# Distributed-Deep-Learning/MiniPs

Hardware: AMD Instinct MI355X
Metric: samples/sec (whole node) Criteo-shaped Wide&Deep BSP at 1/2/4/8 MI355X (higher is better)
Workload: dtype bf16; 1 GPU; global_batch=16384, parallelism=ps-dp1 (bsp; single rank: local shards, no collectives), per_gpu_batch=16384, consistency=bsp, world_size=1, backend=none, lookahead=2

## Files before the change

csrc/kernels/gemm_kernels.h:

```cpp
#pragma once
#include <cstdlib>
#include <stdexcept>
#include <string>

#include "common.h"
#include "kernels.h"

namespace minips_k {

typedef __bf16 v8bf __attribute__((ext_vector_type(8)));
typedef unsigned int v4u __attribute__((ext_vector_type(4)));

constexpr int BM = 128, BN = 128;

template <int BK>
struct Lds {
  static constexpr int ROW = BK + 8;
  static constexpr int TR = BM + 16;
  static constexpr int TILE = (BM * ROW > BK * TR) ? BM * ROW : BK * TR;
  static constexpr int CHUNKS = BM * BK / 8 / 256;
};

__device__ __forceinline__ v4s ds_read_tr16(const bf16_t* p) {
  return __builtin_amdgcn_ds_read_tr16_b64_v4i16((__attribute__((address_space(3))) v4s*)(p));
// ... 443 lines not shown
      const int gr = row0 + R, gk = k0 + 8 * c;
      voff = (gr < rows && gk < kend) ? (uint32_t)(((int64_t)gr * ld + gk) * 2) : kOobOffset;
    } else {
      constexpr int CH = ROWS / 8;
      constexpr int RPI = 64 / CH;
      const int kr = RPI * gi + lane / CH;
      const int c = (lane % CH) ^ swz_k(kr);
      const int gk = k0 + kr, gm = row0 + 8 * c;
      voff = (gk < kend && gm < rows) ? (uint32_t)(((int64_t)gk * ld + gm) * 2) : kOobOffset;
    }
    __builtin_amdgcn_raw_ptr_buffer_load_lds(rsrc, (__attribute__((address_space(3))) void*)(S + gi * 512), 16, voff,
                                             0, 0, 0);
  }
}

template <bool KMAJOR, bool PERM, int ROWS>
__device__ __forceinline__ v8s frag2(const bf16_t* S, int row_base, int ks, int lane) {
  const int g = lane >> 4;
  if (!KMAJOR) {
    const int R = row_base + (lane & 15);
    const int c = (4 * ks + g) ^ ((R >> 1) & 7);
    return *reinterpret_cast<const v8s*>(S + R * BK2 + 8 * c);
  } else {
    const int i = lane & 15, q = i >> 2, p = i & 3;
    const int r0 = 32 * ks + (PERM ? 4 * g : 8 * g) + q;
    const int r1 = 32 * ks + (PERM ? 16 + 4 * g : 8 * g + 4) + q;
    const int ch = (row_base >> 3) + (p >> 1), sub = 4 * (p & 1);
    const v4s lo = ds_read_tr16(S + r0 * ROWS + 8 * (ch ^ swz_k(r0)) + sub);
    const v4s hi = ds_read_tr16(S + r1 * ROWS + 8 * (ch ^ swz_k(r1)) + sub);
    return __builtin_shufflevector(lo, hi, 0, 1, 2, 3, 4, 5, 6, 7);
  }
}

template <int TM, int TN, bool A_KM, bool B_KN, int EPI>
__global__ __launch_bounds__(TM * TN / 64) void gemm_v2_kernel(const bf16_t* __restrict__ A,
                                                               const bf16_t* __restrict__ B, int M, int N, int K,
                                                               int lda, int ldb, int k_chunk, EpiArgs ep) {
  constexpr bool PERM = A_KM && B_KN;
  constexpr int WN = TN / 64, NWAVES = (TM / 64) * (TN / 64);
  constexpr int VM_STAGE = (TM / 8 + TN / 8) / NWAVES;
  __shared__ __attribute__((aligned(1024))) bf16_t smem[2][(TM + TN) * BK2];
  static_assert(sizeof(smem) >= sizeof(float) * NWAVES * kScrFloats, "epilogue scratch must fit the staging LDS");
  const int tid = threadIdx.x, lane = tid & 63, wave = tid >> 6;
  const int wm = wave / WN, wn = wave % WN;
  const int tiles_n = (N + TN - 1) / TN, tiles_m = (M + TM - 1) / TM;
  const int nwg = tiles_m * tiles_n;
  int bid = blockIdx.x, ks = blockIdx.z;
  if (ep.zmap && gridDim.z > 1 && gridDim.y == 1) {
    const int W = nwg * (int)gridDim.z, L = bid + nwg * ks;
    const int xcd = L & 7, q = W >> 3, r = W & 7;
    const int w = (xcd < r ? xcd * (q + 1) : r * (q + 1) + (xcd - r) * q) + (L >> 3);
    ks = w / nwg;
    bid = w - ks * nwg;
  } else if (nwg >= 16) {
    int xcd = bid & 7, q = nwg >> 3, r = nwg & 7;
    int base = xcd < r ? xcd * (q + 1) : r * (q + 1) + (xcd - r) * q;
    bid = base + (bid >> 3);
  }
  const int tm = bid / tiles_n, tn = bid % tiles_n;
  const int m0 = tm * TM, n0 = tn * TN;
  {
    const int z = blockIdx.y, zo = z / ep.inner, zi = z - zo * ep.inner;
    A += zo * ep.sa_o + zi * ep.sa_i;
    B += zo * ep.sb_o + zi * ep.sb_i;
    const int64_t co = zo * ep.sc_o + zi * ep.sc_i + (int64_t)ks * ep.sc_split;
    const bool f32 = EPI == kEpiStoreF32 || EPI == kEpiAtomicF32 || EPI == kEpiAccumF32;
    ep.C = f32 ? (void*)((float*)ep.C + co) : (void*)((bf16_t*)ep.C + co);
  }
  const __amdgpu_buffer_rsrc_t ra = __builtin_amdgcn_make_buffer_rsrc((void*)A, (short)0, 0x7ffffff0, 0x00020000);
  const __amdgpu_buffer_rsrc_t rb = __builtin_amdgcn_make_buffer_rsrc((void*)B, (short)0, 0x7ffffff0, 0x00020000);
  const int kb = ks * k_chunk;
  const int ke = min(K, kb + k_chunk);
  const int nt = ke > kb ? (ke - kb + BK2 - 1) / BK2 : 0;

  v4f acc[4][4];
#pragma unroll
  for (int i = 0; i < 4; ++i)
#pragma unroll
    for (int j = 0; j < 4; ++j) acc[i][j] = v4f{0.f, 0.f, 0.f, 0.f};

  if (nt > 0) {
    dma_tile<A_KM, TM, NWAVES>(ra, lda, m0, kb, M, ke, smem[0], wave, lane);
    dma_tile<B_KN, TN, NWAVES>(rb, ldb, n0, kb, N, ke, smem[0] + TM * BK2, wave, lane);
  }
  for (int t = 0; t < nt; ++t) {
    const int cur = t & 1;
    if (t + 1 < nt) {
      const int k1 = kb + (t + 1) * BK2;
      dma_tile<A_KM, TM, NWAVES>(ra, lda, m0, k1, M, ke, smem[cur ^ 1], wave, lane);
      dma_tile<B_KN, TN, NWAVES>(rb, ldb, n0, k1, N, ke, smem[cur ^ 1] + TM * BK2, wave, lane);
      asm volatile("s_waitcnt vmcnt(%0)" ::"n"(VM_STAGE) : "memory");
    } else {
      asm volatile("s_waitcnt vmcnt(0)" ::: "memory");
    }
    __builtin_amdgcn_s_barrier();
    asm volatile("" ::: "memory");
    const bf16_t* SA = smem[cur];
    const bf16_t* SB = smem[cur] + TM * BK2;
#pragma unroll
    for (int ks = 0; ks < BK2 / 32; ++ks) {
      v8s af[4], bfr[4];
#pragma unroll
      for (int i = 0; i < 4; ++i) af[i] = frag2<A_KM, PERM, TM>(SA, wm * 64 + i * 16, ks, lane);
#pragma unroll
      for (int j = 0; j < 4; ++j) bfr[j] = frag2<B_KN, PERM, TN>(SB, wn * 64 + j * 16, ks, lane);
      if (kSetPrio) __builtin_amdgcn_s_setprio(1);
#pragma unroll
      for (int i = 0; i < 4; ++i)
#pragma unroll
        for (int j = 0; j < 4; ++j)
          acc[i][j] = __builtin_amdgcn_mfma_f32_16x16x32_bf16(__builtin_bit_cast(v8bf, af[i]),
                                                              __builtin_bit_cast(v8bf, bfr[j]), acc[i][j], 0, 0, 0);
      if (kSetPrio) __builtin_amdgcn_s_setprio(0);
    }
    asm volatile("s_waitcnt lgkmcnt(0)" ::: "memory");
    __builtin_amdgcn_s_barrier();
    asm volatile("" ::: "memory");
  }
  if (kLdsEpilogue)
    epilogue_lds<EPI, 4>(acc, ep, M, N, m0 + wm * 64, n0 + wn * 64, lane,
                         reinterpret_cast<float*>(&smem[0][0]) + wave * kScrFloats);
  else
    epilogue<EPI>(acc, ep, M, N, m0, n0, wm, wn, lane);
}

inline int gemm_force_tile() {
  static const int v = [] {
    const char* e = std::getenv("MINIPS_GEMM_TILE");
    return e ? std::atoi(e) : 0;
  }();
  return v;
}

template <bool A_KM, bool B_KN, int EPI>
int launch(const bf16_t* A, const bf16_t* B, int M, int N, int K, int lda, int ldb, int split_k,
                  const EpiArgs& ep, int batch, hipStream_t s) {
  int tiles = ((M + BM - 1) / BM) * ((N + BN - 1) / BN);
  const int64_t a_ext = (int64_t)((A_KM ? K : M) - 1) * lda + (A_KM ? M : K);
  const int64_t b_ext = (int64_t)((B_KN ? K : N) - 1) * ldb + (B_KN ? N : K);
  const bool wgrad = A_KM && B_KN;
  const bool v2_ok = a_ext * 2 < 0x7ff00000ll && b_ext * 2 < 0x7ff00000ll;
  const int force = gemm_force_tile();
  if (force != 1 && v2_ok) {
    const int kper = (K + split_k - 1) / split_k;
    const int kc = (kper + BK2 - 1) / BK2 * BK2;
    const int nsplit = (K + kc - 1) / kc;
    const int64_t work = (int64_t)batch * nsplit;
    const int64_t t256 = work * ((M + 255) / 256) * ((N + 255) / 256);
    const int64_t t128 = work * (int64_t)tiles;
    const double eff256 = (double)t256 / (double)(((t256 + 255) / 256) * 256);
    const double eff128 = (double)t128 / (double)(((t128 + 511) / 512) * 512);
// ... 73 lines not shown
```

minips_amd/_native.py:

```python
from __future__ import annotations

import importlib
import os

_loaded: dict = {}


def _load(name: str, what: str, torch_ext: bool = True):
    if name not in _loaded:
        try:
            if torch_ext:
                import torch

            _loaded[name] = importlib.import_module("minips_amd." + name)
        except Exception as e:
            _loaded[name] = e
    mod = _loaded[name]
    if isinstance(mod, Exception):
        state, fix = ("is not built or failed to load", " (or __graft_entry__.build()).") if torch_ext else \
            ("is not built", ".")
        raise RuntimeError(f"minips_amd.{name} ({what}) {state}: {mod!r}. Run `python tools/build.py`{fix}")
    return mod


# ... 3 lines not shown
        return True
    except RuntimeError:
        return False


def kernels():
    return _load("_kernels", "gfx950 HIP kernels")


def evalk():
    return _load("_evalk", "gfx950 HIP evaluation kernels")


def optk():
    return _load("_optk", "gfx950 HIP gradient-clipping kernels")


def ftrlk():
    return _load("_ftrlk", "gfx950 HIP FTRL-Proximal kernel")


def wdftrlk():
    return _load("_wdftrlk", "gfx950 HIP Adagrad + FTRL-Proximal split-row kernel")


def fmk():
    return _load("_fmk", "gfx950 HIP factorization-machine kernels")


def dfmk():
    return _load("_dfmk", "gfx950 HIP DeepFM interaction-term kernels")


def runtime():
    return _load("_runtime", "C++ PS runtime", torch_ext=False)


def kernels_available() -> bool:
    return _available(kernels)


def evalk_available() -> bool:
    return _available(evalk)


def optk_available() -> bool:
    return _available(optk)


def ftrlk_available() -> bool:
    return _available(ftrlk)


def wdftrlk_available() -> bool:
    return _available(wdftrlk)


def fmk_available() -> bool:
    return _available(fmk)


def dfmk_available() -> bool:
    return _available(dfmk)


def native_dir() -> str:
    return os.path.dirname(os.path.abspath(__file__))
```

minips_amd/models/widedeep.py:

```python
from __future__ import annotations

from dataclasses import dataclass, field

import torch

from .. import ops
from ..ps.comm import Comm
from ..utils import streams
from ..utils.metrics import phase, traced
from .layers import Replayer, SideStream
from .feeder import LookaheadPlans


@dataclass
class WideDeepConfig:
    cards: list = field(default_factory=lambda: list(__import__(
        "minips_amd.data.synthetic", fromlist=["CRITEO_KAGGLE_CARDS"]).CRITEO_KAGGLE_CARDS))
    n_dense: int = 13
    emb_dim: int = 32
    row_width: int = 36
    hidden: tuple = (1024, 512, 256)
    lr_dense: float = 1e-3
    lr_sparse: float = 0.02
    consistency: str = "bsp"
    staleness: int = 0
    transport: str = "auto"
    dense_transport: str | None = None
    max_batch: int = 16384
    seed: int = 0
    bucket_mb: float = 0.0
    wide_optimizer: str = "adagrad"
    wide_alpha: float = 0.1
    wide_beta: float = 1.0
    wide_l1: float = 0.0
    wide_l2: float = 0.0
    wide_grad_scale: float = 1.0
    fm_term: bool = False

    def __post_init__(self):
# ... 6 lines not shown
        if self.wide_optimizer == "ftrl" and self.transport == "onesided":
            raise ValueError("wide_optimizer 'ftrl' needs transport 'collective' (the one-sided owners apply the "
                             "row-wise Adagrad only)")
        if self.fm_term and "onesided" in (self.transport, self.dense_transport):
            raise ValueError("fm_term needs transport 'collective' (the DeepFM term is not built for the one-sided "
                             "transport)")
        if self.fm_term and not 1 <= self.emb_dim <= 64:
            raise ValueError(f"fm_term: emb_dim is {self.emb_dim}, expected 1 <= emb_dim <= 64")

    @property
    def F(self):
        return len(self.cards)

    @property
    def in_dim(self):
        k = self.F * self.emb_dim + self.n_dense + 1
        return (k + 7) // 8 * 8


_PLAN_AT = {1: "dgrad", 2: "dgrad"}
_DENSE_CLOCK_ON_SIDE = False


_K1_ALIGN = 64
_WGRAD_BLOCKS = 256


_DENSE_ON_SIDE = True
_W1_LATE = False
_ADAM_AFTER_DGRAD = True
_ROWIDX = True
_REPLAY = True
_HEAD_DEFER = True


def _wgrad(dH, H, Gw, sink=None):
    return ops.linear_wgrad(dH, H, Gw, blocks=_WGRAD_BLOCKS, defer=sink)


def _align(n, a=8):
    return (n + a - 1) // a * a


def _table_maker(comm, engine):
    from ..engine import create_table

    if engine is not None:
        return lambda kind, **kw: engine.table(engine.create_table(kind, **kw))
    ids = iter(range(1 << 20))
    return lambda kind, **kw: create_table(comm, kind, table_id=next(ids), **kw)


class WideDeep(LookaheadPlans):
    def __init__(self, cfg: WideDeepConfig, comm: Comm, engine=None):
        self.cfg = cfg
        self.comm = comm
        dev = comm.device
        F, D = cfg.F, cfg.emb_dim
        self.num_rows = int(sum(cfg.cards))
        bases = [sum(cfg.cards[:f]) for f in range(F)]
        make = _table_maker(comm, engine)
        onesided = cfg.transport == "onesided"
        self.emb = make("sparse", num_rows=self.num_rows, width=cfg.row_width, optimizer="rowwise_adagrad",
                        lr=cfg.lr_sparse, model=cfg.consistency, staleness=cfg.staleness, transport=cfg.transport,
                        split=D, init_std=0.01, seed=cfg.seed, columns=(bases, cfg.cards), pull_dtype=torch.bfloat16,
                        **({"max_keys": cfg.max_batch * F} if onesided else {}),
                        **(dict(wide_optimizer="ftrl", wide_lr=cfg.wide_alpha, ftrl_beta=cfg.wide_beta, l1=cfg.wide_l1,
                                l2=cfg.wide_l2, ftrl_grad_scale=cfg.wide_grad_scale)
                           if cfg.wide_optimizer == "ftrl" else {}))
        self.emb.shard[:, D:].zero_()
        self.k_in = [cfg.F * cfg.emb_dim + cfg.n_dense, *cfg.hidden[:-1]]
        self.k_pad = [_align(self.k_in[0] + 1, _K1_ALIGN),
                      *self.k_in[1:]]
        self.layout = {}
        off = 0
        for i, n_out in enumerate(cfg.hidden):
            self.layout[f"W{i + 1}"] = (off, (n_out, self.k_pad[i]))
            off += _align(n_out * self.k_pad[i], 64)
            if i > 0:
                self.layout[f"b{i + 1}"] = (off, (n_out,))
                off += _align(n_out, 64)
        self.layout["w4"] = (off, (cfg.hidden[-1] + 8,))
        off += cfg.hidden[-1] + 8
        self.n_params = off
        starts = [self.layout[f"W{i + 1}"][0] for i in range(len(cfg.hidden))]
        bucketed = cfg.bucket_mb > 0 and cfg.dense_transport == "collective" and comm.world > 1
        self.dense = make("dense", n_params=self.n_params, optimizer="adam", lr=cfg.lr_dense, model=cfg.consistency,
                          staleness=cfg.staleness, transport=cfg.dense_transport,
                          **(dict(buckets=starts, bucket_mb=cfg.bucket_mb) if bucketed else {}))
        self._wbucket = [self.dense.bucket_for_layer(x) for x in starts] if bucketed else None
        self.dense.load_full(self._init_dense(dev))
        self._bufs = {}
        self._side = SideStream(dev)
        self._replay = Replayer(self._side) if self._side.stream is not None else None

    def _init_dense(self, dev):
        g = torch.Generator(device="cpu")
        g.manual_seed(self.cfg.seed + 17)
        full = torch.zeros(self.n_params, dtype=torch.float32)
        for i in range(len(self.cfg.hidden)):
            w = self.view(full, f"W{i + 1}")
            ops.kaiming_uniform_(w[:, : self.k_in[i]], self.k_in[i], g)
            w[:, self.k_in[i]:] = 0
        h = self.cfg.hidden[-1]
        ops.kaiming_uniform_(self.view(full, "w4")[:h], h, g)
        return full.to(dev)

    def view(self, buf: torch.Tensor, name: str) -> torch.Tensor:
        key = (buf.data_ptr(), buf.dtype, name)
        views = self.__dict__.setdefault("_views", {})
        v = views.get(key)
        if v is None:
            off, shape = self.layout[name]
            n = 1
            for s in shape:
                n *= s
            v = buf[off: off + n].view(shape)
            if buf.is_cuda:
                if len(views) > 256:
                    views.clear()
                views[key] = v
        return v

    def _buffers(self, B):
        if B not in self._bufs:
            dev, cfg = self.comm.device, self.cfg
            bf = dict(dtype=torch.bfloat16, device=dev)
            h1, h2, h3 = cfg.hidden

            X = torch.zeros(B, self.k_pad[0], **bf)
            X[:, self.k_in[0]] = 1.0

            self._bufs[B] = dict(
                X=X, H1=torch.empty(B, h1, **bf), H2=torch.empty(B, h2, **bf),
                H3=torch.empty(B, h3, **bf), dH3=torch.empty(B, h3, **bf), dH2=torch.empty(B, h2, **bf),
                dH1=torch.empty(B, h1, **bf),
                dX=torch.empty(B, cfg.F * cfg.emb_dim, **bf),
                wide=torch.empty(B, dtype=torch.float32, device=dev),
                dwide=torch.empty(B, dtype=torch.float32, device=dev),
                loss=torch.zeros(1, dtype=torch.float32, device=dev),
            )
            if cfg.fm_term:
                self._bufs[B]["S"] = torch.empty(B, cfg.emb_dim, dtype=torch.float32, device=dev)
        return self._bufs[B]

    def _forward(self, b, P):
        ops.linear_fwd(b["X"], self.view(P, "W1"), None, "relu", out=b["H1"])
        ops.linear_fwd(b["H1"], self.view(P, "W2"), self.view(P, "b2"), "relu", out=b["H2"])
        ops.linear_fwd(b["H2"], self.view(P, "W3"), self.view(P, "b3"), "relu", out=b["H3"])

    def forward(self, dense, keys, rows, plan):
        B = dense.shape[0]
        b = self._buffers(B)
        pend_side = self.__dict__.pop("_side_pending", None)
        if pend_side is not None:
            streams.current(self.comm.device).wait_event(pend_side[1])
        P = self.dense.get()
        F, D = self.cfg.F, self.cfg.emb_dim
        ops.wd_assemble(dense, rows, plan.inv, F, D, b["X"], b["wide"], ones_col=self.k_in[0])
        if self.cfg.fm_term:
            ops.wd_fm_forward(b["X"], F, D, b["wide"], b["S"])
        self._forward(b, P)
        h = self.cfg.hidden[-1]
        w4 = self.view(P, "w4").float()
        return b["H3"].float() @ w4[:h] + w4[h] + b["wide"]

    def _eval_buffers(self, B):
        bufs = self.__dict__.setdefault("_ebufs", {})
        if B not in bufs:
            dev, cfg = self.comm.device, self.cfg
            bf = dict(dtype=torch.bfloat16, device=dev)
            X = torch.zeros(B, self.k_pad[0], **bf)
            X[:, self.k_in[0]] = 1.0
            bufs[B] = dict(X=X, wide=torch.empty(B, dtype=torch.float32, device=dev),
                           **{f"H{i + 1}": torch.empty(B, n, **bf) for i, n in enumerate(cfg.hidden)})
            if cfg.fm_term:
                bufs[B]["S"] = torch.empty(B, cfg.emb_dim, dtype=torch.float32, device=dev)
        return bufs[B]

    def evaluate(self, batches, evaluator=None) -> dict:
        from ..utils.evalmetrics import BinaryEvaluator

        cfg = self.cfg
        if "onesided" in (cfg.transport, cfg.dense_transport):
            raise NotImplementedError("WideDeep.evaluate: the onesided transport is not supported (its Gets move the "
                                      "SSP gate's staleness statistics and need a clock); evaluate on 'collective'")
        ev = evaluator if evaluator is not None else BinaryEvaluator(self.comm.device)
        F, D, h = cfg.F, cfg.emb_dim, cfg.hidden[-1]
        pend_side = self.__dict__.get("_side_pending")
        if pend_side is not None:
            streams.current(self.comm.device).wait_event(pend_side[1])
        P = self.dense.get()
        w4 = self.view(P, "w4")
        for dense, keys, labels in batches:
            b = self._eval_buffers(dense.shape[0])
            rows, plan = self.emb.get(keys, plan=self.emb.plan(keys))
            ops.wd_assemble(dense, rows, plan.inv, F, D, b["X"], b["wide"], ones_col=self.k_in[0])
            if cfg.fm_term:
                ops.wd_fm_forward(b["X"], F, D, b["wide"], b["S"])
            self._forward(b, P)
            ev.update_head(b["H3"], w4[:h], w4[h:h + 1], b["wide"], labels)
        ev.reduce(self.comm)
        return ev.result()

    @traced("wd.train_step")
    def train_step(self, dense, keys, labels, next_keys=None, next_on_plan_stream: bool = False) -> torch.Tensor:
        cfg = self.cfg
        B = dense.shape[0]
        F, D = cfg.F, cfg.emb_dim
        h = cfg.hidden[-1]
        b = self._buffers(B)
        plan = self._take_plan(keys)

        def issue_next(point):
            if next_keys is not None and point == _PLAN_AT[min(2, self.comm.world)]:
                nk = next_keys() if callable(next_keys) else next_keys
                self.prefetch(nk, keys_on_plan_stream=next_on_plan_stream)

        with phase("wd.plan_next"):
            issue_next("start")
        pend_side = self.__dict__.pop("_side_pending", None)
        if pend_side is not None and pend_side[0] is not None:
            streams.current(self.comm.device).wait_event(pend_side[0])
        ph = phase("wd.get_assemble")
        ph.__enter__()
        src = self.emb.get_source(keys, plan=plan)
        if src is not None:
            plan, table, index, base = src
            rowidx = plan.csr[4] if plan.csr is not None and len(plan.csr) >= 5 and _ROWIDX else None
            ops.wd_assemble_tab(dense, table, index, base, plan.inv, F, D, b["X"], b["wide"], ones_col=self.k_in[0],
                                zero=b["loss"], rowidx=rowidx)
        else:
            rows, plan = self.emb.get(keys, plan=plan)
            ops.wd_assemble(dense, rows, plan.inv, F, D, b["X"], b["wide"], ones_col=self.k_in[0], zero=b["loss"])
        if cfg.fm_term:
            ops.wd_fm_forward(b["X"], F, D, b["wide"], b["S"])
        if pend_side is not None:
            streams.current(self.comm.device).wait_event(pend_side[1])
        ph.__exit__(None, None, None)
        ph = phase("wd.fwd_head")
        ph.__enter__()
        G = self.dense.grad
        P = self.dense.get()
        scale = 1.0 / (B * self.comm.world)
        w4, gw4 = self.view(P, "w4"), self.view(G, "w4")
        sink = self.dense.slab_sink() if hasattr(self.dense, "slab_sink") else None
        side = self._side
        defer = _HEAD_DEFER and side.stream is not None
        rp = self._replay if (self._replay is not None and _REPLAY and self._wbucket is None
                              and streams.DELAY_US <= 0 and not torch.cuda.is_current_stream_capturing()) else None
        key = (B, P.data_ptr(), G.data_ptr(), sink is not None, defer)
        if rp is not None:
            rp(("fwd",) + key, lambda: self._forward(b, P))
        else:
            self._forward(b, P)
        ops.wd_head(b["H3"], w4[:h], w4[h:h + 1], b["wide"], labels, b["dH3"], gw4[:h], gw4[h:h + 1],
                    b["dwide"], b["loss"], self.view(G, "b3"), scale, defer_fold=defer)
        ph.__exit__(None, None, None)
        ph = phase("wd.bwd_dense")
        ph.__enter__()
        issue_next("head")
        fold = (B, h, gw4[:h], gw4[h:h + 1], b["loss"], self.view(G, "b3")) if defer else None
        if rp is not None:
            rp(("bwd",) + key, lambda: self._backward_chain(b, P, G, sink, side, fold))
        else:
            self._backward_chain(b, P, G, sink, side, fold)
        sorted_rows = plan.csr is not None and len(plan.csr) >= 3 and plan.csr[2] is not None
        if sorted_rows:
            ops.linear_dgrad(b["dH1"], self.view(P, "W1"), n_cols=F * D, out=b["dX"].view(B * F, D),
                             perm=plan.csr[2], seg=D)
        else:
            ops.linear_dgrad(b["dH1"], self.view(P, "W1"), n_cols=F * D, out=b["dX"])
        w_read = side.point() if _ADAM_AFTER_DGRAD and self.comm.world == 1 else None
        if cfg.fm_term:
            ops.wd_fm_backward(b["X"], b["S"], b["dwide"], b["dX"], F, D, perm=plan.csr[2] if sorted_rows else None)
        if _W1_LATE:
            with side.fork():
                _wgrad(b["dH1"], b["X"], self.view(G, "W1"), sink)
        pipe = getattr(self.dense, "pipe", None)
        dense_early = _DENSE_CLOCK_ON_SIDE and pipe is not None and pipe.async_ and side.stream is not None
        if dense_early:
            with side.fork():
                self.dense.add()
                self.dense.clock()
        issue_next("dgrad")
        ph.__exit__(None, None, None)
        ph = phase("wd.emb_push")
        ph.__enter__()
        dXe = b["dX"].view(B * F, D) if sorted_rows else b["dX"]
        self.emb.add_lookup_grads(plan, dXe, b["dwide"], F, D, sorted_rows=sorted_rows)
        self.emb.clock()
        issue_next("push")
        ph.__exit__(None, None, None)
        ph = phase("wd.dense_clock")
        ph.__enter__()
# ... 60 lines not shown
```

minips_amd/ops/__init__.py:

```python
from __future__ import annotations

import math

import torch

from .._native import dfmk, evalk, fmk, ftrlk, kernels, optk, wdftrlk

EPI_STORE_F32 = 0
EPI_ATOMIC_F32 = 1
EPI_BIAS_RELU_BF16 = 2
EPI_BIAS_BF16 = 3
EPI_STORE_BF16 = 4
EPI_RELU_MASK_BF16 = 5
EPI_BIAS_GELU_BF16 = 6
EPI_BIAS_GELU_AUX_BF16 = 7
EPI_GELU_GRAD_BF16 = 8
EPI_PERM_ROWS_BF16 = 9
EPI_BIAS_GELU_DAUX_BF16 = 13
EPI_MUL_AUX_BF16 = 14
_L2E = 1.4426950408889634


def _gelu_grad(u):
    k, c = 0.7978845608, 0.044715
    t = torch.tanh(k * (u + c * u ** 3))
    return 0.5 * (1 + t) + 0.5 * u * (1 - t * t) * k * (1 + 3 * c * u * u)


def _gpu(t: torch.Tensor) -> bool:
    return t.is_cuda


_NO_STRIDES: list = []
_REC = None


class recording:

    def __init__(self, lst):
# ... 502 lines not shown
                                  zero, rowidx)
        return X, wide_logit
    U = int(inv.max()) + 1 if inv.numel() else 0
    rows = table[index[:U] - base].to(torch.bfloat16)
    return wd_assemble(dense, rows, inv, F, D, X, wide_logit, ones_col, zero)


def wd_head(H, w, b0, wide_logit, labels, dH, dw, db, dwide, loss_sum, dH_colsum=None, grad_scale=1.0,
            defer_fold=False):
    if _gpu(H):
        kernels().wd_head(H, w, b0, wide_logit, labels, dH, dw, db, dwide, loss_sum, dH_colsum, float(grad_scale),
                          bool(defer_fold))
        return
    h = H.float()
    z = h @ w.float() + b0.float() + wide_logit
    y = (labels > 0.5).float()
    p = torch.sigmoid(z)
    dz = (p - y) * grad_scale
    dwide.copy_(dz)
    db += dz.sum()
    loss_sum += (torch.clamp_min(z, 0) - z * y + torch.log1p(torch.exp(-z.abs()))).sum()
    g = torch.where(h > 0, dz.unsqueeze(1) * w.float().unsqueeze(0), torch.zeros_like(h)).to(torch.bfloat16)
    dH.copy_(g)
    dw += (dz.unsqueeze(1) * h).sum(0)
    if dH_colsum is not None:
        dH_colsum += g.float().sum(0)


def wd_head_fold(B, Hd, dw, db, loss_sum, dH_colsum=None):
    if _gpu(dw):
        (kernels() if _REC is None else _REC.lst).wd_head_fold(int(B), int(Hd), dw, db, loss_sum, dH_colsum)


def _wd_fm_check(X, F, D):
    if not 1 <= D <= 64 or F < 1:
        raise RuntimeError(f"wd_fm: D is {D} and F is {F}, expected 1 <= D <= 64 and F >= 1")
    if X.dim() != 2 or X.shape[1] < F * D:
        raise RuntimeError(f"wd_fm: X has shape {tuple(X.shape)}, expected [B, >= F * D = {F * D}]")


def wd_fm_forward(X, F, D, wide, S=None, blocks=0):
    F, D, B = int(F), int(D), X.shape[0]
    if S is None:
        S = torch.empty(B, D, dtype=torch.float32, device=X.device)
    if _gpu(X):
        dfmk().wd_fm_forward(X, F, D, wide, S, int(blocks))
        return S
    _wd_fm_check(X, F, D)
    v = X[:, : F * D].float().reshape(B, F, D)
    s = v.sum(1)
    S.copy_(s)
    wide += 0.5 * (s * s - (v * v).sum(1)).sum(1)
    return S


def wd_fm_backward(X, S, dwide, dX, F, D, perm=None, blocks=0):
    F, D, B = int(F), int(D), X.shape[0]
    if _gpu(X):
        dfmk().wd_fm_backward(X, S, dwide, perm, dX, F, D, int(blocks))
        return dX
    _wd_fm_check(X, F, D)
    n = B * F
    if dX.numel() != n * D or not dX.is_contiguous():
        raise RuntimeError(f"wd_fm_backward: dX {tuple(dX.shape)}, expected {n * D} contiguous elements")
    v = X[:, : F * D].float().reshape(n, D)
    dx = dX.view(n, D)
# ... 600 lines not shown
```

Before: 48.70 million samples/s.

## Fuse layer-3 GEMM with Wide&Deep head and BCE loss into one tail kernel

Adds a HIP kernel that computes the last hidden layer (H2·W3ᵀ + b3, ReLU), the output head, the BCE loss and its gradient in one pass. H3 is never written to global memory, and per-block partial sums (dw4, db4, loss, b3 column sums) are reduced by a separate fold kernel launched on the side stream. This removes the layer-3 GEMM launch, the H3 round trip and the separate head kernel. In exchange, each block recomputes the full 256-wide N tile, and the design relies on a partials buffer and on restricted shapes (N a multiple of 64, at most 256). The GEMM main loop is factored into a macro so the new kernel can reuse it.

```diff
diff --git a/csrc/bindings/wdtail_py.cpp b/csrc/bindings/wdtail_py.cpp
--- /dev/null
+++ b/csrc/bindings/wdtail_py.cpp
@@ -0,0 +1,108 @@
+#include <ATen/hip/impl/HIPGuardImplMasqueradingAsCUDA.h>
+#include <ATen/hip/impl/HIPStreamMasqueradingAsCUDA.h>
+#include <torch/extension.h>
+
+#include "../kernels/wdtail.h"
+#include "tensor_access.h"
+
+namespace {
+
+using namespace minips_access;
+using OptTensor = c10::optional<at::Tensor>;
+using DeviceGuard = c10::hip::HIPGuardMasqueradingAsCUDA;
+
+void check_n(int64_t N, const char* what) {
+  TORCH_CHECK(N >= 64 && N <= minips_k::kTailMaxN && N % 64 == 0, what, " ", N, ", expected a multiple of 64 up to ",
+              minips_k::kTailMaxN);
+}
+
+int64_t wd_tail(const at::Tensor& H2, const at::Tensor& W3, const at::Tensor& b3, const at::Tensor& w4,
+                const at::Tensor& b4, const at::Tensor& wide, const at::Tensor& labels, at::Tensor& dH3,
+                at::Tensor& dwide, at::Tensor& partials, const OptTensor& H3_out, double grad_scale, int64_t tile) {
+  TORCH_CHECK(H2.dim() == 2 && W3.dim() == 2, "H2 and W3 must be matrices ([B, K] and [N, K])");
+  const int64_t B = H2.size(0), K = H2.size(1), N = W3.size(0);
+  check_n(N, "W3 has N =");
+  TORCH_CHECK(tile == 0 || tile == 64 || tile == 128, "tile is ", tile, ", expected 0, 64 or 128");
+  TORCH_CHECK(B >= 1, "H2 has shape ", H2.sizes(), ", expected at least one row");
+  TORCH_CHECK(W3.size(1) == K, "W3 has shape ", W3.sizes(), ", expected [N, ", K, "] (H2's columns)");
+  const int64_t ldh = B > 1 ? H2.stride(0) : K, ldw = W3.stride(0);
+  DeviceGuard gd(gpu_of(H2, "H2"));
+  const bf16_t* hp = dev_rows<bf16_t>(H2, "H2", B, K);
+  const bf16_t* wp = dev_rows<bf16_t>(W3, "W3", N, K);
+  TORCH_CHECK(minips_k::tail_shape_ok(B, N, K, ldh, ldw), "H2 has shape ", H2.sizes(), " (ld ", ldh, "), W3 ",
+              W3.sizes(), " (ld ", ldw, "): K and both leading dimensions must be multiples of 8, below 2 GiB each");
+  aligned16(H2, "H2");
+  aligned16(W3, "W3");
+  TORCH_CHECK(b3.dim() == 1 && b3.numel() == N, "b3 has shape ", b3.sizes(), ", expected [", N, "]");
+  TORCH_CHECK(w4.dim() == 1 && w4.numel() == N, "w4 has shape ", w4.sizes(), ", expected [", N, "]");
+  TORCH_CHECK(b4.dim() == 1 && b4.numel() == 1, "b4 has shape ", b4.sizes(), ", expected [1]");
+  TORCH_CHECK(wide.dim() == 1 && wide.numel() == B, "wide has shape ", wide.sizes(), ", expected [", B, "]");
+  TORCH_CHECK(labels.dim() == 1 && labels.numel() == B, "labels has shape ", labels.sizes(), ", expected [", B, "]");
+  TORCH_CHECK(dH3.dim() == 2 && dH3.size(0) == B && dH3.size(1) == N, "dH3 has shape ", dH3.sizes(), ", expected [", B,
+              ", ", N, "]");
+  TORCH_CHECK(dwide.dim() == 1 && dwide.numel() == B, "dwide has shape ", dwide.sizes(), ", expected [", B, "]");
+  const int64_t rows = minips_k::tail_blocks(B, tile == 0 ? minips_k::kTailDefaultTM : (int)tile), NP = 2 * N + 2;
+  TORCH_CHECK(partials.dim() == 2 && partials.size(1) == NP && partials.size(0) >= rows, "partials has shape ",
+              partials.sizes(), ", expected [>= ", rows, ", ", NP, "]");
+  if (present(H3_out))
+    TORCH_CHECK(H3_out->dim() == 2 && H3_out->size(0) == B && H3_out->size(1) == N, "H3_out has shape ",
+                H3_out->sizes(), ", expected [", B, ", ", N, "]");
+  const bf16_t* b3p = dev<bf16_t>(b3, "b3", N);
+  const bf16_t* w4p = dev<bf16_t>(w4, "w4", N);
+  const bf16_t* b4p = dev<bf16_t>(b4, "b4", 1);
+  const float* wdp = dev<float>(wide, "wide", B);
+  const float* lbp = dev<float>(labels, "labels", B);
+  bf16_t* dhp = dev<bf16_t>(dH3, "dH3", B * N);
+  float* dwp = dev<float>(dwide, "dwide", B);
+  float* pp = dev<float>(partials, "partials", rows * NP);
+  bf16_t* h3p = dev_opt<bf16_t>(H3_out, "H3_out", B * N);
+  aligned16(dH3, "dH3");
+  if (present(H3_out)) aligned16(*H3_out, "H3_out");
+  const auto d = H2.device();
+  TORCH_CHECK(W3.device() == d && b3.device() == d && w4.device() == d && b4.device() == d && wide.device() == d &&
+                  labels.device() == d && dH3.device() == d && dwide.device() == d && partials.device() == d &&
+                  (!present(H3_out) || H3_out->device() == d),
+              "W3, b3, w4, b4, wide, labels, dH3, dwide, partials and H3_out must be on H2's device");
+  return minips_k::wd_tail(hp, ldh, wp, ldw, b3p, w4p, b4p, wdp, lbp, dhp, dwp, pp, h3p, B, (int)N, (int)K,
+                           (float)grad_scale, (int)tile, stream_of(H2));
+}
+
+void wd_tail_fold(const at::Tensor& partials, int64_t nblocks, int64_t N, at::Tensor& dw4, at::Tensor& db4,
+                  at::Tensor& loss_sum, const OptTensor& colsum_b3) {
+  check_n(N, "N is");
+  TORCH_CHECK(nblocks >= 1 && nblocks <= minips_k::kTailMaxBlocks, "nblocks is ", nblocks,
+              ", expected 1 <= nblocks <= ", minips_k::kTailMaxBlocks);
+  const int64_t NP = 2 * N + 2;
+  TORCH_CHECK(partials.dim() == 2 && partials.size(1) == NP && partials.size(0) >= nblocks, "partials has shape ",
+              partials.sizes(), ", expected [>= nblocks = ", nblocks, ", ", NP, "]");
+  TORCH_CHECK(dw4.dim() == 1 && dw4.numel() == N, "dw4 has shape ", dw4.sizes(), ", expected [", N, "]");
+  TORCH_CHECK(db4.dim() == 1 && db4.numel() == 1, "db4 has shape ", db4.sizes(), ", expected [1]");
+  TORCH_CHECK(loss_sum.dim() == 1 && loss_sum.numel() == 1, "loss_sum has shape ", loss_sum.sizes(), ", expected [1]");
+  if (present(colsum_b3))
+    TORCH_CHECK(colsum_b3->dim() == 1 && colsum_b3->numel() == N, "colsum_b3 has shape ", colsum_b3->sizes(),
+                ", expected [", N, "]");
+  DeviceGuard gd(gpu_of(partials, "partials"));
+  const float* pp = dev<float>(partials, "partials", nblocks * NP);
+  float* dwp = dev<float>(dw4, "dw4", N);
+  float* dbp = dev<float>(db4, "db4", 1);
+  float* lp = dev<float>(loss_sum, "loss_sum", 1);
+  float* cp = dev_opt<float>(colsum_b3, "colsum_b3", N);
+  const auto d = partials.device();
+  TORCH_CHECK(dw4.device() == d && db4.device() == d && loss_sum.device() == d &&
+                  (!present(colsum_b3) || colsum_b3->device() == d),
+              "dw4, db4, loss_sum and colsum_b3 must be on partials' device");
+  minips_k::wd_tail_fold(pp, (int)nblocks, (int)N, dwp, dbp, lp, cp, stream_of(partials));
+}
+
+}
+
+PYBIND11_MODULE(TORCH_EXTENSION_NAME, m) {
+  m.doc() = "minips_amd fused Wide & Deep MLP tail: layer-3 GEMM + head + BCE forward/backward (gfx950)";
+  m.def("wd_tail", &wd_tail, py::arg("H2"), py::arg("W3"), py::arg("b3"), py::arg("w4"), py::arg("b4"),
+        py::arg("wide"), py::arg("labels"), py::arg("dH3"), py::arg("dwide"), py::arg("partials"), py::arg("H3_out"),
+        py::arg("grad_scale"), py::arg("tile"));
+  m.def("wd_tail_fold", &wd_tail_fold, py::arg("partials"), py::arg("nblocks"), py::arg("N"), py::arg("dw4"),
+        py::arg("db4"), py::arg("loss_sum"), py::arg("colsum_b3"));
+  m.attr("MAX_N") = minips_k::kTailMaxN;
+  m.attr("MAX_BLOCKS") = minips_k::kTailMaxBlocks;
+}
diff --git a/csrc/kernels/gemm_kernels.h b/csrc/kernels/gemm_kernels.h
--- a/csrc/kernels/gemm_kernels.h
+++ b/csrc/kernels/gemm_kernels.h
@@ -499,6 +499,41 @@
   }
 }
 
+#define MINIPS_GEMM_V2_MAIN_LOOP(TM, TN, ra, rb, lda, ldb, M, N, m0, n0, kb, ke, nt, smem, wave, lane, wm, wn, acc) \
+  if (nt > 0) {                                                                                                    \
+    dma_tile<A_KM, TM, NWAVES>(ra, lda, m0, kb, M, ke, smem[0], wave, lane);                                       \
+    dma_tile<B_KN, TN, NWAVES>(rb, ldb, n0, kb, N, ke, smem[0] + TM * BK2, wave, lane);                            \
+  }                                                                                                                \
+  for (int t = 0; t < nt; ++t) {                                                                                   \
+    const int cur = t & 1;                                                                                         \
+    if (t + 1 < nt) {                                                                                              \
+      const int k1 = kb + (t + 1) * BK2;                                                                           \
+      dma_tile<A_KM, TM, NWAVES>(ra, lda, m0, k1, M, ke, smem[cur ^ 1], wave, lane);                               \
+      dma_tile<B_KN, TN, NWAVES>(rb, ldb, n0, k1, N, ke, smem[cur ^ 1] + TM * BK2, wave, lane);                    \
+                                                                       \
+      asm volatile("s_waitcnt vmcnt(%0)" ::"n"(VM_STAGE) : "memory");                                              \
+    } else {                                                                                                       \
+      asm volatile("s_waitcnt vmcnt(0)" ::: "memory");                                                             \
+    }                                                                                                              \
+    __builtin_amdgcn_s_barrier();                                                                                  \
+    asm volatile("" ::: "memory");                                                                                 \
+    const bf16_t* SA = smem[cur];                                                                                  \
+    const bf16_t* SB = smem[cur] + TM * BK2;                                                                       \
+    _Pragma("unroll") for (int ks = 0; ks < BK2 / 32; ++ks) {                                                      \
+      v8s af[4], bfr[4];                                                                                           \
+      _Pragma("unroll") for (int i = 0; i < 4; ++i) af[i] = frag2<A_KM, PERM, TM>(SA, wm * 64 + i * 16, ks, lane); \
+      _Pragma("unroll") for (int j = 0; j < 4; ++j) bfr[j] = frag2<B_KN, PERM, TN>(SB, wn * 64 + j * 16, ks, lane); \
+      if (kSetPrio) __builtin_amdgcn_s_setprio(1);                \
+      _Pragma("unroll") for (int i = 0; i < 4; ++i) _Pragma("unroll") for (int j = 0; j < 4; ++j) acc[i][j] =      \
+          __builtin_amdgcn_mfma_f32_16x16x32_bf16(__builtin_bit_cast(v8bf, af[i]), __builtin_bit_cast(v8bf, bfr[j]), \
+                                                  acc[i][j], 0, 0, 0);                                             \
+      if (kSetPrio) __builtin_amdgcn_s_setprio(0);                                                                 \
+    }                                                                                                              \
+    asm volatile("s_waitcnt lgkmcnt(0)" ::: "memory");                                                             \
+    __builtin_amdgcn_s_barrier();                     \
+    asm volatile("" ::: "memory");                                                                                 \
+  }
+
 template <int TM, int TN, bool A_KM, bool B_KN, int EPI>
 __global__ __launch_bounds__(TM * TN / 64) void gemm_v2_kernel(const bf16_t* __restrict__ A,
                                                                const bf16_t* __restrict__ B, int M, int N, int K,
@@ -546,44 +581,7 @@
 #pragma unroll
     for (int j = 0; j < 4; ++j) acc[i][j] = v4f{0.f, 0.f, 0.f, 0.f};
 
-  if (nt > 0) {
-    dma_tile<A_KM, TM, NWAVES>(ra, lda, m0, kb, M, ke, smem[0], wave, lane);
-    dma_tile<B_KN, TN, NWAVES>(rb, ldb, n0, kb, N, ke, smem[0] + TM * BK2, wave, lane);
-  }
-  for (int t = 0; t < nt; ++t) {
-    const int cur = t & 1;
-    if (t + 1 < nt) {
-      const int k1 = kb + (t + 1) * BK2;
-      dma_tile<A_KM, TM, NWAVES>(ra, lda, m0, k1, M, ke, smem[cur ^ 1], wave, lane);
-      dma_tile<B_KN, TN, NWAVES>(rb, ldb, n0, k1, N, ke, smem[cur ^ 1] + TM * BK2, wave, lane);
-      asm volatile("s_waitcnt vmcnt(%0)" ::"n"(VM_STAGE) : "memory");
-    } else {
-      asm volatile("s_waitcnt vmcnt(0)" ::: "memory");
-    }
-    __builtin_amdgcn_s_barrier();
-    asm volatile("" ::: "memory");
-    const bf16_t* SA = smem[cur];
-    const bf16_t* SB = smem[cur] + TM * BK2;
-#pragma unroll
-    for (int ks = 0; ks < BK2 / 32; ++ks) {
-      v8s af[4], bfr[4];
-#pragma unroll
-      for (int i = 0; i < 4; ++i) af[i] = frag2<A_KM, PERM, TM>(SA, wm * 64 + i * 16, ks, lane);
-#pragma unroll
-      for (int j = 0; j < 4; ++j) bfr[j] = frag2<B_KN, PERM, TN>(SB, wn * 64 + j * 16, ks, lane);
-      if (kSetPrio) __builtin_amdgcn_s_setprio(1);
-#pragma unroll
-      for (int i = 0; i < 4; ++i)
-#pragma unroll
-        for (int j = 0; j < 4; ++j)
-          acc[i][j] = __builtin_amdgcn_mfma_f32_16x16x32_bf16(__builtin_bit_cast(v8bf, af[i]),
-                                                              __builtin_bit_cast(v8bf, bfr[j]), acc[i][j], 0, 0, 0);
-      if (kSetPrio) __builtin_amdgcn_s_setprio(0);
-    }
-    asm volatile("s_waitcnt lgkmcnt(0)" ::: "memory");
-    __builtin_amdgcn_s_barrier();
-    asm volatile("" ::: "memory");
-  }
+  MINIPS_GEMM_V2_MAIN_LOOP(TM, TN, ra, rb, lda, ldb, M, N, m0, n0, kb, ke, nt, smem, wave, lane, wm, wn, acc)
   if (kLdsEpilogue)
     epilogue_lds<EPI, 4>(acc, ep, M, N, m0 + wm * 64, n0 + wn * 64, lane,
                          reinterpret_cast<float*>(&smem[0][0]) + wave * kScrFloats);
diff --git a/csrc/kernels/wdtail.h b/csrc/kernels/wdtail.h
--- /dev/null
+++ b/csrc/kernels/wdtail.h
@@ -0,0 +1,30 @@
+#pragma once
+
+#include <hip/hip_runtime.h>
+#include <stdint.h>
+
+namespace minips_k {
+
+constexpr int kTailMaxN = 256;
+constexpr int kTailMaxBlocks = 256;
+constexpr int kTailDefaultTM = 128;
+
+inline bool tail_shape_ok(int64_t B, int64_t N, int64_t K, int64_t ldh, int64_t ldw) {
+  constexpr int64_t kMaxElems = 0x7ff00000ll >> 1;
+  return B >= 1 && N >= 64 && N <= kTailMaxN && N % 64 == 0 && K >= 8 && K % 8 == 0 && ldh >= K && ldw >= K &&
+         ldh % 8 == 0 && ldw % 8 == 0 && (B - 1) * ldh + K < kMaxElems && (N - 1) * ldw + K < kMaxElems;
+}
+
+inline int tail_blocks(int64_t B, int tm) {
+  const int64_t tiles = (B + tm - 1) / tm;
+  return (int)(tiles < kTailMaxBlocks ? tiles : kTailMaxBlocks);
+}
+
+int wd_tail(const uint16_t* H2, int64_t ldh, const uint16_t* W3, int64_t ldw, const uint16_t* b3, const uint16_t* w4,
+            const uint16_t* b4, const float* wide, const float* labels, uint16_t* dH3, float* dwide, float* partials,
+            uint16_t* H3_out, int64_t B, int N, int K, float grad_scale, int tm, hipStream_t stream);
+
+void wd_tail_fold(const float* partials, int nblocks, int N, float* dw4, float* db4, float* loss_sum,
+                  float* colsum_b3, hipStream_t stream);
+
+}
diff --git a/csrc/kernels/wdtail.hip b/csrc/kernels/wdtail.hip
--- /dev/null
+++ b/csrc/kernels/wdtail.hip
@@ -0,0 +1,261 @@
+#include "wdtail.h"
+
+#include <stdexcept>
+#include <string>
+
+#include "gemm_kernels.h"
+
+namespace minips_k {
+namespace {
+
+constexpr int kTailTN = 256;
+
+__device__ __forceinline__ void tail_store_slice(const v4f (&v)[4], float* __restrict__ scr, bf16_t* __restrict__ dst,
+                                                 int B, int N, int row0, int nb, int lane) {
+  const int col_l = lane & 15, row_q = (lane >> 4) * 4;
+#pragma unroll
+  for (int j = 0; j < 4; ++j)
+#pragma unroll
+    for (int r = 0; r < 4; ++r) scr[(row_q + r) * kScrPitch + j * 16 + col_l] = v[j][r];
+  __builtin_amdgcn_wave_barrier();
+#pragma unroll
+  for (int ro = 0; ro < 2; ++ro) {
+    const int rr = ro * 8 + (lane >> 3), c8 = (lane & 7) * 8;
+    const int row = row0 + rr, col = nb + c8;
+    const float4 lo = *reinterpret_cast<const float4*>(scr + rr * kScrPitch + c8);
+    const float4 hi = *reinterpret_cast<const float4*>(scr + rr * kScrPitch + c8 + 4);
+    if (row >= B || col >= N) continue;
+    auto pk = [](float a, float b) { return (__float_as_uint(a) >> 16) | (__float_as_uint(b) & 0xffff0000u); };
+    *reinterpret_cast<uint4*>(dst + (int64_t)row * N + col) =
+        make_uint4(pk(lo.x, lo.y), pk(lo.z, lo.w), pk(hi.x, hi.y), pk(hi.z, hi.w));
+  }
+  __builtin_amdgcn_wave_barrier();
+}
+
+template <int TM>
+__global__ __launch_bounds__(TM * 4, 2) void wd_tail_kernel(const bf16_t* __restrict__ H2,
+                                                         const bf16_t* __restrict__ W3, int B, int N, int K, int ldh,
+                                                         int ldw,
+                                                         const bf16_t* __restrict__ b3, const bf16_t* __restrict__ w4,
+                                                         const bf16_t* __restrict__ b4, const float* __restrict__ wide,
+                                                         const float* __restrict__ labels, bf16_t* __restrict__ dH3,
+                                                         float* __restrict__ dwide, float* __restrict__ partials,
+                                                         bf16_t* __restrict__ H3_out, float scale, int ntiles) {
+  constexpr bool A_KM = false, B_KN = false, PERM = false;
+  constexpr int TN = kTailTN, WMS = TM / 64, NWAVES = WMS * (TN / 64);
+  constexpr int VM_STAGE = (TM / 8 + TN / 8) / NWAVES;
+  __shared__ __attribute__((aligned(1024))) bf16_t smem[2][(TM + TN) * BK2];
+  const int tid = threadIdx.x, lane = tid & 63, wave = tid >> 6;
+  const int wm = wave / (TN / 64), wn = wave % (TN / 64);
+  const int col_l = lane & 15, row_q = (lane >> 4) * 4;
+  float* const lds = reinterpret_cast<float*>(&smem[0][0]);
+  float* const scr = lds + wave * kScrFloats;
+  float* const zpart = lds + NWAVES * kScrFloats;
+  float* const dzs = zpart + 4 * TM;
+  float* const red = dzs + TM;
+  float* const red_s = red + 2 * WMS * TN;
+  static_assert(sizeof(smem) >= sizeof(float) * (NWAVES * kScrFloats + 5 * TM + 2 * WMS * TN + 2 * NWAVES),
+                "the epilogue's scratch must fit the staging LDS");
+
+  const __amdgpu_buffer_rsrc_t ra = __builtin_amdgcn_make_buffer_rsrc((void*)H2, (short)0, 0x7ffffff0, 0x00020000);
+  const __amdgpu_buffer_rsrc_t rb = __builtin_amdgcn_make_buffer_rsrc((void*)W3, (short)0, 0x7ffffff0, 0x00020000);
+  const int nt = (K + BK2 - 1) / BK2;
+
+  float wc[4], bc[4], dwl[4], csl[4];
+#pragma unroll
+  for (int j = 0; j < 4; ++j) {
+    const int col = wn * 64 + j * 16 + col_l;
+    wc[j] = col < N ? bf2f(w4[col]) : 0.f;
+    bc[j] = col < N ? bf2f(b3[col]) : 0.f;
+    dwl[j] = 0.f;
+    csl[j] = 0.f;
+  }
+  const float bias4 = bf2f(b4[0]);
+  float dbl = 0.f, lossl = 0.f;
+
+  for (int tile = blockIdx.x; tile < ntiles; tile += gridDim.x) {
+    const int m0 = tile * TM;
+    v4f acc[4][4];
+#pragma unroll
+    for (int i = 0; i < 4; ++i)
+#pragma unroll
+      for (int j = 0; j < 4; ++j) acc[i][j] = v4f{0.f, 0.f, 0.f, 0.f};
+    MINIPS_GEMM_V2_MAIN_LOOP(TM, TN, ra, rb, ldh, ldw, B, N, m0, 0, 0, K, nt, smem, wave, lane, wm, wn, acc)
+
+#pragma unroll
+    for (int i = 0; i < 4; ++i)
+#pragma unroll
+      for (int j = 0; j < 4; ++j)
+#pragma unroll
+        for (int r = 0; r < 4; r += 2) {
+          const uint32_t p = pack_bf2(fmaxf(acc[i][j][r] + bc[j], 0.f), fmaxf(acc[i][j][r + 1] + bc[j], 0.f));
+          acc[i][j][r] = __uint_as_float(p << 16);
+          acc[i][j][r + 1] = __uint_as_float(p & 0xffff0000u);
+        }
+    if (H3_out) {
+#pragma unroll
+      for (int i = 0; i < 4; ++i)
+        tail_store_slice(acc[i], scr, H3_out, B, N, m0 + wm * 64 + i * 16, wn * 64, lane);
+    }
+#pragma unroll
+    for (int i = 0; i < 4; ++i)
+#pragma unroll
+      for (int r = 0; r < 4; ++r) {
+        float s = 0.f;
+#pragma unroll
+        for (int j = 0; j < 4; ++j) s += acc[i][j][r] * wc[j];
+        s += __shfl_xor(s, 1, 64);
+        s += __shfl_xor(s, 2, 64);
+        s += __shfl_xor(s, 4, 64);
+        s += __shfl_xor(s, 8, 64);
+        if (col_l == 0) zpart[wn * TM + wm * 64 + i * 16 + row_q + r] = s;
+      }
+    __syncthreads();
+    if (tid < TM) {
+      const int row = m0 + tid;
+      float dz = 0.f;
+      if (row < B) {
+        const float z = ((zpart[tid] + zpart[TM + tid]) + zpart[2 * TM + tid]) + zpart[3 * TM + tid];
+        const float zz = z + bias4 + wide[row];
+        const float label = labels[row] > 0.5f ? 1.f : 0.f;
+        const float p = sigmoidf_(zz);
+        dz = (p - label) * scale;
+        dwide[row] = dz;
+        dbl += dz;
+        lossl += fmaxf(zz, 0.f) - zz * label + log1pf(__expf(-fabsf(zz)));
+      }
+      dzs[tid] = dz;
+    }
+    __syncthreads();
+
+#pragma unroll
+    for (int i = 0; i < 4; ++i) {
+      const float4 d4 = *reinterpret_cast<const float4*>(dzs + wm * 64 + i * 16 + row_q);
+      const float dz[4] = {d4.x, d4.y, d4.z, d4.w};
+      v4f g[4];
+#pragma unroll
+      for (int j = 0; j < 4; ++j)
+#pragma unroll
+        for (int r = 0; r < 4; r += 2) {
+          const float h0 = acc[i][j][r], h1 = acc[i][j][r + 1];
+          const uint32_t p = pack_bf2(h0 > 0.f ? dz[r] * wc[j] : 0.f, h1 > 0.f ? dz[r + 1] * wc[j] : 0.f);
+          g[j][r] = __uint_as_float(p << 16);
+          g[j][r + 1] = __uint_as_float(p & 0xffff0000u);
+          dwl[j] += dz[r] * h0;
+          dwl[j] += dz[r + 1] * h1;
+          csl[j] += g[j][r];
+          csl[j] += g[j][r + 1];
+        }
+      tail_store_slice(g, scr, dH3, B, N, m0 + wm * 64 + i * 16, wn * 64, lane);
+    }
+    __syncthreads();
+  }
+
+#pragma unroll
+  for (int j = 0; j < 4; ++j) {
+    dwl[j] += __shfl_xor(dwl[j], 16, 64);
+    dwl[j] += __shfl_xor(dwl[j], 32, 64);
+    csl[j] += __shfl_xor(csl[j], 16, 64);
+    csl[j] += __shfl_xor(csl[j], 32, 64);
+    if (lane < 16) {
+      red[wm * TN + wn * 64 + j * 16 + lane] = dwl[j];
+      red[(WMS + wm) * TN + wn * 64 + j * 16 + lane] = csl[j];
+    }
+  }
+  dbl = warp_sum(dbl);
+  lossl = warp_sum(lossl);
+  if (lane == 0) {
+    red_s[wave] = dbl;
+    red_s[NWAVES + wave] = lossl;
+  }
+  __syncthreads();
+  float* const prow = partials + (int64_t)blockIdx.x * (2 * N + 2);
+  for (int c = tid; c < N; c += TM * 4) {
+    float a = 0.f, b = 0.f;
+#pragma unroll
+    for (int w = 0; w < WMS; ++w) {
+      a += red[w * TN + c];
+      b += red[(WMS + w) * TN + c];
+    }
+    prow[c] = a;
+    prow[N + c] = b;
+  }
+  if (tid == 0) {
+    float a = 0.f, b = 0.f;
+#pragma unroll
+    for (int w = 0; w < NWAVES; ++w) {
+      a += red_s[w];
+      b += red_s[NWAVES + w];
+    }
+    prow[2 * N] = a;
+    prow[2 * N + 1] = b;
+  }
+}
+
+constexpr int kTailFoldCols = 32, kTailFoldChunks = 16;
+__global__ __launch_bounds__(kTailFoldCols* kTailFoldChunks) void wd_tail_fold_kernel(
+    const float* __restrict__ partials, int nb, int N, float* dw, float* colsum, float* db, float* loss_sum) {
+  __shared__ float red[kTailFoldChunks][kTailFoldCols + 1];
+  const int NP = 2 * N + 2;
+  const int cl = threadIdx.x % kTailFoldCols, ch = threadIdx.x / kTailFoldCols;
+  const int c = blockIdx.x * kTailFoldCols + cl;
+  const int per = (nb + kTailFoldChunks - 1) / kTailFoldChunks;
+  const int r0 = ch * per, r1 = min(nb, r0 + per);
+  float acc = 0.f;
+  if (c < NP) {
+    for (int r = r0; r < r1; r += 8) {
+      float v[8];
+#pragma unroll
+      for (int k = 0; k < 8; ++k) v[k] = r + k < r1 ? partials[(int64_t)(r + k) * NP + c] : 0.f;
+#pragma unroll
+      for (int k = 0; k < 8; ++k) acc += v[k];
+    }
+  }
+  red[ch][cl] = acc;
+  __syncthreads();
+  if (ch != 0 || c >= NP) return;
+  float tot = 0.f;
+#pragma unroll
+  for (int k = 0; k < kTailFoldChunks; ++k) tot += red[k][cl];
+  if (c < N) dw[c] += tot;
+  else if (c < 2 * N) {
+    if (colsum) colsum[c - N] += tot;
+  } else if (c == 2 * N) *db += tot;
+  else *loss_sum += tot;
+}
+
+}
+
+int wd_tail(const uint16_t* H2, int64_t ldh, const uint16_t* W3, int64_t ldw, const uint16_t* b3, const uint16_t* w4,
+            const uint16_t* b4, const float* wide, const float* labels, uint16_t* dH3, float* dwide, float* partials,
+            uint16_t* H3_out, int64_t B, int N, int K, float grad_scale, int tm, hipStream_t stream) {
+  if (B <= 0) return 0;
+  if (!tail_shape_ok(B, N, K, ldh, ldw))
+    throw std::runtime_error("wd_tail: B " + std::to_string(B) + ", N " + std::to_string(N) + ", K " +
+                             std::to_string(K) + ": N must be a multiple of 64 up to 256, K a multiple of 8");
+  if (tm == 0) tm = kTailDefaultTM;
+  if (tm != 64 && tm != 128) throw std::runtime_error("wd_tail: tile " + std::to_string(tm) + ", expected 64 or 128");
+  const int ntiles = (int)((B + tm - 1) / tm), grid = tail_blocks(B, tm);
+  if (tm == 64)
+    hipLaunchKernelGGL(wd_tail_kernel<64>, grid, 256, 0, stream, H2, W3, (int)B, N, K, (int)ldh, (int)ldw, b3, w4, b4,
+                       wide, labels, dH3, dwide, partials, H3_out, grad_scale, ntiles);
+  else
+    hipLaunchKernelGGL(wd_tail_kernel<128>, grid, 512, 0, stream, H2, W3, (int)B, N, K, (int)ldh, (int)ldw, b3, w4, b4,
+                       wide, labels, dH3, dwide, partials, H3_out, grad_scale, ntiles);
+  MINIPS_HIP_CHECK(hipGetLastError());
+  return grid;
+}
+
+void wd_tail_fold(const float* partials, int nblocks, int N, float* dw4, float* db4, float* loss_sum,
+                  float* colsum_b3, hipStream_t stream) {
+  if (nblocks <= 0) return;
+  if (N < 64 || N > kTailMaxN || N % 64 != 0 || nblocks > kTailMaxBlocks)
+    throw std::runtime_error("wd_tail_fold: N " + std::to_string(N) + ", nblocks " + std::to_string(nblocks) +
+                             ": N must be a multiple of 64 up to 256, nblocks at most 256");
+  const int NP = 2 * N + 2;
+  hipLaunchKernelGGL(wd_tail_fold_kernel, (NP + kTailFoldCols - 1) / kTailFoldCols, kTailFoldCols * kTailFoldChunks, 0,
+                     stream, partials, nblocks, N, dw4, colsum_b3, db4, loss_sum);
+  MINIPS_HIP_CHECK(hipGetLastError());
+}
+
+}
diff --git a/minips_amd/_native.py b/minips_amd/_native.py
--- a/minips_amd/_native.py
+++ b/minips_amd/_native.py
@@ -59,6 +59,10 @@
     return _load("_dfmk", "gfx950 HIP DeepFM interaction-term kernels")
 
 
+def wdtailk():
+    return _load("_wdtailk", "gfx950 HIP fused Wide & Deep MLP tail kernels")
+
+
 def runtime():
     return _load("_runtime", "C++ PS runtime", torch_ext=False)
 
@@ -91,5 +95,9 @@
     return _available(dfmk)
 
 
+def wdtailk_available() -> bool:
+    return _available(wdtailk)
+
+
 def native_dir() -> str:
     return os.path.dirname(os.path.abspath(__file__))
diff --git a/minips_amd/models/widedeep.py b/minips_amd/models/widedeep.py
--- a/minips_amd/models/widedeep.py
+++ b/minips_amd/models/widedeep.py
@@ -4,7 +4,7 @@
 
 import torch
 
-from .. import ops
+from .. import _native, ops
 from ..ps.comm import Comm
 from ..utils import streams
 from ..utils.metrics import phase, traced
@@ -77,6 +77,8 @@
 _ROWIDX = True
 _REPLAY = True
 _HEAD_DEFER = True
+_TAIL_FUSED = True
+_TAIL_TILE = 0
 
 
 def _wgrad(dH, H, Gw, sink=None):
@@ -138,6 +140,8 @@
         self._bufs = {}
         self._side = SideStream(dev)
         self._replay = Replayer(self._side) if self._side.stream is not None else None
+        h = cfg.hidden[-1]
+        self._tail_ok = self._side.stream is not None and h % 64 == 0 and h <= 256 and _native.wdtailk_available()
 
     def _init_dense(self, dev):
         g = torch.Generator(device="cpu")
@@ -167,7 +171,7 @@
                 views[key] = v
         return v
 
-    def _buffers(self, B):
+    def _buffers(self, B, with_h3=True):
         if B not in self._bufs:
             dev, cfg = self.comm.device, self.cfg
             bf = dict(dtype=torch.bfloat16, device=dev)
@@ -178,7 +182,7 @@
 
             self._bufs[B] = dict(
                 X=X, H1=torch.empty(B, h1, **bf), H2=torch.empty(B, h2, **bf),
-                H3=torch.empty(B, h3, **bf), dH3=torch.empty(B, h3, **bf), dH2=torch.empty(B, h2, **bf),
+                dH3=torch.empty(B, h3, **bf), dH2=torch.empty(B, h2, **bf),
                 dH1=torch.empty(B, h1, **bf),
                 dX=torch.empty(B, cfg.F * cfg.emb_dim, **bf),
                 wide=torch.empty(B, dtype=torch.float32, device=dev),
@@ -187,7 +191,16 @@
             )
             if cfg.fm_term:
                 self._bufs[B]["S"] = torch.empty(B, cfg.emb_dim, dtype=torch.float32, device=dev)
-        return self._bufs[B]
+            if self._tail_ok:
+                self._bufs[B]["partials"] = torch.empty(256, 2 * h3 + 2, dtype=torch.float32, device=dev)
+        b = self._bufs[B]
+        if with_h3 and "H3" not in b:
+            b["H3"] = torch.empty(B, self.cfg.hidden[-1], dtype=torch.bfloat16, device=self.comm.device)
+        return b
+
+    def _forward_hidden(self, b, P):
+        ops.linear_fwd(b["X"], self.view(P, "W1"), None, "relu", out=b["H1"])
+        ops.linear_fwd(b["H1"], self.view(P, "W2"), self.view(P, "b2"), "relu", out=b["H2"])
 
     def _forward(self, b, P):
         ops.linear_fwd(b["X"], self.view(P, "W1"), None, "relu", out=b["H1"])
@@ -254,7 +267,8 @@
         B = dense.shape[0]
         F, D = cfg.F, cfg.emb_dim
         h = cfg.hidden[-1]
-        b = self._buffers(B)
+        tail = _TAIL_FUSED and self._tail_ok
+        b = self._buffers(B, with_h3=not tail)
         plan = self._take_plan(keys)
 
         def issue_next(point):
@@ -294,18 +308,27 @@
         defer = _HEAD_DEFER and side.stream is not None
         rp = self._replay if (self._replay is not None and _REPLAY and self._wbucket is None
                               and streams.DELAY_US <= 0 and not torch.cuda.is_current_stream_capturing()) else None
-        key = (B, P.data_ptr(), G.data_ptr(), sink is not None, defer)
+        key = (B, P.data_ptr(), G.data_ptr(), sink is not None, defer, tail)
+        fwd = self._forward_hidden if tail else self._forward
         if rp is not None:
-            rp(("fwd",) + key, lambda: self._forward(b, P))
-        else:
-            self._forward(b, P)
-        ops.wd_head(b["H3"], w4[:h], w4[h:h + 1], b["wide"], labels, b["dH3"], gw4[:h], gw4[h:h + 1],
-                    b["dwide"], b["loss"], self.view(G, "b3"), scale, defer_fold=defer)
+            rp(("fwd",) + key, lambda: fwd(b, P))
+        else:
+            fwd(b, P)
+        if tail:
+            nblocks = ops.wd_tail(b["H2"], self.view(P, "W3"), self.view(P, "b3"), w4[:h], w4[h:h + 1], b["wide"],
+                                  labels, b["dH3"], b["dwide"], b["partials"], scale, tile=_TAIL_TILE)
+        else:
+            ops.wd_head(b["H3"], w4[:h], w4[h:h + 1], b["wide"], labels, b["dH3"], gw4[:h], gw4[h:h + 1],
+                        b["dwide"], b["loss"], self.view(G, "b3"), scale, defer_fold=defer)
         ph.__exit__(None, None, None)
         ph = phase("wd.bwd_dense")
         ph.__enter__()
         issue_next("head")
-        fold = (B, h, gw4[:h], gw4[h:h + 1], b["loss"], self.view(G, "b3")) if defer else None
+        fold = (B, h, gw4[:h], gw4[h:h + 1], b["loss"], self.view(G, "b3")) if defer and not tail else None
+        if tail:
+            with side.fork():
+                ops.wd_tail_fold(b["partials"], nblocks, h, gw4[:h], gw4[h:h + 1], b["loss"], self.view(G, "b3"))
+            defer = True
         if rp is not None:
             rp(("bwd",) + key, lambda: self._backward_chain(b, P, G, sink, side, fold))
         else:
diff --git a/minips_amd/ops/__init__.py b/minips_amd/ops/__init__.py
--- a/minips_amd/ops/__init__.py
+++ b/minips_amd/ops/__init__.py
@@ -4,7 +4,7 @@
 
 import torch
 
-from .._native import dfmk, evalk, fmk, ftrlk, kernels, optk, wdftrlk
+from .._native import dfmk, evalk, fmk, ftrlk, kernels, optk, wdftrlk, wdtailk
 
 EPI_STORE_F32 = 0
 EPI_ATOMIC_F32 = 1
@@ -573,6 +573,30 @@
         (kernels() if _REC is None else _REC.lst).wd_head_fold(int(B), int(Hd), dw, db, loss_sum, dH_colsum)
 
 
+def wd_tail(H2, W3, b3, w4, b4, wide, labels, dH3, dwide, partials, grad_scale=1.0, H3_out=None, tile=0):
+    if _gpu(H2):
+        return wdtailk().wd_tail(H2, W3, b3, w4, b4, wide, labels, dH3, dwide, partials, H3_out, float(grad_scale),
+                                 int(tile))
+    N = W3.shape[0]
+    H3 = linear_fwd(H2, W3, b3, "relu", out=H3_out)
+    partials[0].zero_()
+    wd_head(H3, w4, b4, wide, labels, dH3, partials[0, :N], partials[0, 2 * N:2 * N + 1], dwide,
+            partials[0, 2 * N + 1:], partials[0, N:2 * N], grad_scale)
+    return 1
+
+
+def wd_tail_fold(partials, nblocks, N, dw4, db4, loss_sum, colsum_b3=None):
+    if _gpu(partials):
+        wdtailk().wd_tail_fold(partials, int(nblocks), int(N), dw4, db4, loss_sum, colsum_b3)
+        return
+    p = partials[:nblocks].sum(0) if nblocks > 1 else partials[0]
+    dw4 += p[:N]
+    if colsum_b3 is not None:
+        colsum_b3 += p[N:2 * N]
+    db4 += p[2 * N]
+    loss_sum += p[2 * N + 1]
+
+
 def _wd_fm_check(X, F, D):
     if not 1 <= D <= 64 or F < 1:
         raise RuntimeError(f"wd_fm: D is {D} and F is {F}, expected 1 <= D <= 64 and F >= 1")
```

After: 48.82 million samples/s, median of 4. No clear change (+0.2%).
